# spkelle2/simple_mip_solver

Hardware: AMD Instinct MI355X
Metric: node LP-relaxations/s (higher is better)
Workload: dtype f64

## Files before the change

simple_mip_solver_amd/csrc/lp_kernel.hip.h:

```cpp
#pragma once
#include <type_traits>
#include <hip/hip_runtime.h>
#include <stdint.h>

namespace mipx {

constexpr double kPTol = 1e-7;
constexpr double kDTol = 1e-7;
constexpr double kPivTol = 1e-9;
constexpr double kBTol = 1e-9;
constexpr double kMReport = 1e10;

struct LpArgs {
    int m = 0, n = 0;
    const double *A = nullptr, *b = nullptr, *c = nullptr;
    size_t A_stride = 0, b_stride = 0, c_stride = 0;
    const double *l = nullptr, *u = nullptr;
    const int8_t *vstat_in = nullptr;
    const int32_t *slot = nullptr;
    const double *anchor_T = nullptr, *anchor_vec = nullptr;
    const int32_t *anchor_idx = nullptr;
    const int32_t *anchor_sel = nullptr;
    const double *atab_T = nullptr, *atab_vec = nullptr;
    const int32_t *atab_idx = nullptr;
// ... 192 lines not shown
    const unsigned lm = wave_min_u32(hi == hm ? lo : 0xffffffffu);
    kmin = __hiloint2double((int)hm, (int)lm);
    return wave_pick(valid & (hi == hm) & (lo == lm), payload);
}
__device__ __forceinline__ double uniform_f64(double v) {
    const int lo = __builtin_amdgcn_readfirstlane(__double2loint(v));
    const int hi = __builtin_amdgcn_readfirstlane(__double2hiint(v));
    return __hiloint2double(hi, lo);
}
__device__ __forceinline__ double readlane_f64(double v, int l) {
    const int lo = __builtin_amdgcn_readlane(__double2loint(v), l);
    const int hi = __builtin_amdgcn_readlane(__double2hiint(v), l);
    return __hiloint2double(hi, lo);
}
__device__ __forceinline__ double swz16_f64(double v) {
    const int lo = __builtin_amdgcn_ds_swizzle(__double2loint(v), 0x401f);
    const int hi = __builtin_amdgcn_ds_swizzle(__double2hiint(v), 0x401f);
    return __hiloint2double(hi, lo);
}
__device__ __forceinline__ double xor32_f64(double v) { return __shfl_xor(v, 32, 64); }
__device__ __forceinline__ double xor8_f64(double v) { return dpp_f64<0x128, 0xf>(v); }
__device__ __forceinline__ double xor4_f64(double v) {
    int lo = __builtin_amdgcn_update_dpp(__double2loint(v), __double2loint(v), 0x104, 0xf, 0x5, false);
    int hi = __builtin_amdgcn_update_dpp(__double2hiint(v), __double2hiint(v), 0x104, 0xf, 0x5, false);
    lo = __builtin_amdgcn_update_dpp(lo, __double2loint(v), 0x114, 0xf, 0xa, false);
    hi = __builtin_amdgcn_update_dpp(hi, __double2hiint(v), 0x114, 0xf, 0xa, false);
    return __hiloint2double(hi, lo);
}
__device__ __forceinline__ double xor2_f64(double v) { return dpp_f64<0x4e, 0xf>(v); }
__device__ __forceinline__ double xor1_f64(double v) { return dpp_f64<0xb1, 0xf>(v); }
#define MIPX_ROWSUM_STEP(arr_, h_, dist_, xch_)                                             \
    do {                                                                                    \
        const bool up_ = (lane & (dist_)) != 0;                                             \
        _Pragma("unroll") for (int k_ = 0; k_ < (h_); k_++) {                               \
            const double send_ = up_ ? arr_[k_] : arr_[k_ + (h_)];                          \
            const double keep_ = up_ ? arr_[k_ + (h_)] : arr_[k_];                          \
            arr_[k_] = keep_ + xch_(send_);                                                 \
        }                                                                                   \
    } while (0)
#define MIPX_ROWSUMS(arr_, rp_)                                                             \
    do {                                                                                    \
        if ((rp_) == 32) {                                                                  \
            MIPX_ROWSUM_STEP(arr_, 16, 32, xor32_f64);                                      \
            MIPX_ROWSUM_STEP(arr_, 8, 16, swz16_f64);                                       \
            MIPX_ROWSUM_STEP(arr_, 4, 8, xor8_f64);                                         \
            MIPX_ROWSUM_STEP(arr_, 2, 4, xor4_f64);                                         \
            MIPX_ROWSUM_STEP(arr_, 1, 2, xor2_f64);                                         \
            arr_[0] = arr_[0] + xor1_f64(arr_[0]);                                          \
        } else {                                                                            \
            MIPX_ROWSUM_STEP(arr_, 8, 32, xor32_f64);                                       \
            MIPX_ROWSUM_STEP(arr_, 4, 16, swz16_f64);                                       \
            MIPX_ROWSUM_STEP(arr_, 2, 8, xor8_f64);                                         \
            MIPX_ROWSUM_STEP(arr_, 1, 4, xor4_f64);                                         \
            arr_[0] = arr_[0] + xor2_f64(arr_[0]);                                          \
            arr_[0] = arr_[0] + xor1_f64(arr_[0]);                                          \
        }                                                                                   \
    } while (0)
__device__ __forceinline__ int rowsum_row(int lane, int rp) {
    const int r16 = ((lane & 32) ? 8 : 0) | ((lane & 16) ? 4 : 0) | ((lane & 8) ? 2 : 0) | ((lane & 4) ? 1 : 0);
    return rp == 32 ? 2 * r16 + ((lane & 2) ? 1 : 0) : r16;
}

struct alignas(16) MailA {
    int win;
    int lvmeta;
    double x;
};
struct alignas(16) MailB {
    int q;
    int ev;
    double pinv;
};

template <int NW, int R, int C, int MP>
struct Smem {
    static constexpr int NP = 16 * C;
    alignas(16) double row[NP];
    double alpha[4 * NW * R];
    double lo[NP];
    double up[NP];
    double va[NP];
    double vb[NP];
    double d[NP];
    double key[NP];
    double cvec[NP];
    double beta0[MP];
    double ba[4 * NW * R];
    double bb[4 * NW * R];
    double wgt[4 * NW * R];
    double tau[4 * NW * R];
    MailA mbA;
    MailB mbB;
    int bvar[MP];
    int meta[NP];
    int nvar[NP];
    int side[NP];
    int wlist[NP];
    int nw;
    int nfake0;
    double objv;
    int dive_code;
    int seq;
    int pos[NP + MP];
    int8_t wantb[NP + MP];
    int8_t atup[NP + MP];
#ifdef MIPX_KPROF
    unsigned long long prof[16];
#endif
};
__device__ __forceinline__ void read_mail(const MailA &mb, int &win, int &lvmeta, double &x) {
    const int4 v = *reinterpret_cast<const int4 *>(&mb);
    win = __builtin_amdgcn_readfirstlane(v.x);
    lvmeta = __builtin_amdgcn_readfirstlane(v.y);
    x = __hiloint2double(__builtin_amdgcn_readfirstlane(v.w), __builtin_amdgcn_readfirstlane(v.z));
}
__device__ __forceinline__ void read_mail(const MailB &mb, int &q, int &ev, double &pinv) {
    const int4 v = *reinterpret_cast<const int4 *>(&mb);
    q = __builtin_amdgcn_readfirstlane(v.x);
    ev = __builtin_amdgcn_readfirstlane(v.y);
    pinv = __hiloint2double(__builtin_amdgcn_readfirstlane(v.w), __builtin_amdgcn_readfirstlane(v.z));
}

#define MIPX_PICK(dst_, arr_, n_, k_)                                                       \
    do {                                                                                    \
        dst_ = arr_[0];                                                                     \
        _Pragma("unroll") for (int t_ = 1; t_ < n_; t_++) dst_ = (k_) == t_ ? arr_[t_] : dst_; \
    } while (0)
template <int C>
struct RowArr {
    double v[C];
    __device__ __forceinline__ double &operator[](int j) { return v[j]; }
    __device__ __forceinline__ const double &operator[](int j) const { return v[j]; }
};
#define MIPX_ROW(ii_) (grp + NG * (ii_))
#define MIPX_COL(jj_) (32 * ((jj_) >> 1) + 2 * cl + ((jj_)&1))
#define MIPX_PUBLISH_COL(q_)                                                                \
    do {                                                                                    \
        const int qjj_ = 2 * ((q_) >> 5) + ((q_)&1);                                        \
        if (cl == (((q_)&31) >> 1)) {                                                       \
            if constexpr (kVecT) {                                                          \
                _Pragma("unroll") for (int ii = 0; ii < R; ii++) s.alpha[MIPX_ROW(ii)] = T[ii][qjj_]; \
            } else {                                                                        \
                _Pragma("unroll") for (int jj = 0; jj < C; jj++) if (jj == qjj_) {          \
                    _Pragma("unroll") for (int ii = 0; ii < R; ii++) s.alpha[MIPX_ROW(ii)] = T[ii][jj]; \
                }                                                                           \
            }                                                                               \
        }                                                                                   \
         \
         \
        if (lane == 0) __hip_atomic_fetch_add(&s.seq, 1, __ATOMIC_RELEASE, __HIP_MEMORY_SCOPE_WORKGROUP); \
        __builtin_amdgcn_fence(__ATOMIC_RELEASE, "wavefront");                              \
        __builtin_amdgcn_wave_barrier();                                                    \
        __builtin_amdgcn_fence(__ATOMIC_ACQUIRE, "wavefront");                              \
        _Pragma("unroll") for (int ii = 0; ii < R; ii++) al[ii] = s.alpha[MIPX_ROW(ii)];    \
    } while (0)
#define MIPX_AWAIT_COL(target_)                                                             \
    do {                                                                                    \
        while (__hip_atomic_load(&s.seq, __ATOMIC_ACQUIRE, __HIP_MEMORY_SCOPE_WORKGROUP) < (target_)) \
            __builtin_amdgcn_s_sleep(1);                                                    \
    } while (0)
#define MIPX_EXTRACT_ROW(r_)                                                                \
    do {                                                                                    \
        const int rl_ = (r_) / NG;                                                          \
        if (grp == (r_) % NG) {                                                             \
            _Pragma("unroll") for (int ii = 0; ii < R; ii++) if (ii == rl_) {               \
                _Pragma("unroll") for (int jj = 0; jj < C; jj++) s.row[MIPX_COL(jj)] = T[ii][jj]; \
            }                                                                               \
        }                                                                                   \
    } while (0)
#define MIPX_ROW_LDS(jj_) s.row[MIPX_COL(jj_)]
#define MIPX_ROW_REG(jj_) rw[jj_]
#define MIPX_UPDATE_T(r_, q_, pinv_, rowsrc_)                                               \
    do {                                                                                    \
        const int rg_ = (r_) % NG, rl_ = (r_) / NG;                                         \
        const int qcl_ = ((q_)&31) >> 1, qjj_ = 2 * ((q_) >> 5) + ((q_)&1);                 \
        double rh[C];                                                                       \
        _Pragma("unroll") for (int jj = 0; jj < C; jj++) rh[jj] = rowsrc_(jj) * (pinv_);    \
        _Pragma("unroll") for (int ii = 0; ii < R; ii++) {                                  \
            _Pragma("unroll") for (int jj = 0; jj < C; jj++)                                \
                T[ii][jj] = fma(-al[ii], rh[jj], T[ii][jj]);                                \
        }                                                                                   \
        if (cl == qcl_) {                                   \
            if constexpr (kVecT) {                                                          \
                _Pragma("unroll") for (int ii = 0; ii < R; ii++) T[ii][qjj_] = -al[ii] * (pinv_); \
// ... 270 lines not shown
        const double *rowp[R];
#pragma unroll
        for (int ii = 0; ii < R; ii++) {
            const int r = min(MIPX_ROW(ii), m > 0 ? m - 1 : 0);
            if (CUTS && r >= m0) rowp[ii] = g.cut_pi + (size_t)cids[r - m0] * n;
            else rowp[ii] = tsrc + (size_t)r * n;
        }
        if ((n & 1) == 0 && n >= 2) {
            int poff[C / 2];
#pragma unroll
            for (int pp = 0; pp < C / 2; pp++) poff[pp] = min(32 * pp + 2 * cl, n - 2);
#pragma unroll
            for (int ii = 0; ii < R; ii++) {
                const double *arow = rowp[ii];
#pragma unroll
                for (int pp = 0; pp < C / 2; pp++) {
                    const double2 v = m > 0 ? *reinterpret_cast<const double2 *>(arow + poff[pp]) : double2{0.0, 0.0};
                    T[ii][2 * pp] = v.x;
                    T[ii][2 * pp + 1] = v.y;
                }
            }
        } else {
#pragma unroll
            for (int ii = 0; ii < R; ii++) {
                const double *arow = rowp[ii];
#pragma unroll
                for (int jj = 0; jj < C; jj++) T[ii][jj] = m > 0 ? arow[min(MIPX_COL(jj), n - 1)] : 0.0;
            }
        }
    }
    {
        static_assert(NT >= NP + MP, "one staging element per thread");
        const int ic = min(tid, m > 0 ? m - 1 : 0), jc = min(tid, n - 1), vc = min(tid, nv - 1);
        double g_b0;
        if (CUTS && ic >= m0) g_b0 = g.cut_pi0[cids[ic - m0]];
        else g_b0 = anchored ? avec[n + ic] : (m > 0 ? gb[ic] : 0.0);
        const int g_bv = anchored ? aidx[n + ic] : n + ic;
        const double g_d = anchored ? avec[jc] : gc[jc];
        const int g_nv = anchored ? aidx[jc] : jc;
        const double g_lo = lk[jc], g_up = uk[jc];
        const double g_c = gc[jc];
        const int8_t g_st = vin ? vin[vc] : (int8_t)0;
        if (tid < MP) {
            s.beta0[tid] = tid < m ? (anchored ? g_b0 : -g_b0) : 0.0;
            s.bvar[tid] = tid < m ? g_bv : -1;
        }
        if (tid < NP) {
            s.d[tid] = tid < n ? g_d : 0.0;
            s.nvar[tid] = tid < n ? g_nv : -1;
            s.lo[tid] = tid < n ? g_lo : 0.0;
            s.up[tid] = tid < n ? g_up : 0.0;
            s.va[tid] = 0.0;
            s.vb[tid] = 0.0;
            s.cvec[tid] = tid < n ? g_c : 0.0;
        }
        if (tid < NP + MP) {
            const int8_t st = tid < nv ? g_st : (int8_t)0;
            s.wantb[tid] = st == 1;
            s.atup[tid] = st == 2;
            s.pos[tid] = -1;
        }
    }
    int ci[PJ];
    bool cv[PJ], che[PJ];
    double ccl[PJ], ccr[PJ];
#pragma unroll
    for (int kk = 0; kk < PJ; kk++) { ci[kk] = 0; cv[kk] = false; che[kk] = true; ccl[kk] = 0.0; ccr[kk] = 0.0; }
    if (DIVE && ctl && g.dive) {
#pragma unroll
        for (int kk = 0; kk < PJ; kk++) {
            const int k = lane + 64 * kk;
            cv[kk] = k < g.n_int;
            ci[kk] = g.int_idx[cv[kk] ? k : 0];
        }
        if (g.rule != 0) {
#pragma unroll
            for (int kk = 0; kk < PJ; kk++) {
                che[kk] = g.has_entry[ci[kk]] != 0;
                ccl[kk] = g.cost_l[ci[kk]];
                ccr[kk] = g.cost_r[ci[kk]];
            }
        }
    }
    if (tid == 0) s.seq = 0;
    if (DIVE && g.dive_preset && tid < g.dive) {
        g.status[(size_t)node + (size_t)(tid + 1) * (size_t)g.dive_off] = -1;
        g.dive_var[(size_t)tid * (size_t)g.dive_off + node] = -1;
    }
    if (g.zero16 != nullptr && node == 0 && tid < 4) g.zero16[tid] = 0;
    KPROF_SETUP_MARK(9);
    __syncthreads();
    KPROF_SETUP_MARK(10);
    for (int j = tid; j < NP; j += NT) {
        const int v = s.nvar[j];
        if (j < n) s.pos[v] = j;
        const bool fix = j < n && v < n && s.lo[v < n && v >= 0 ? v : 0] == s.up[v < n && v >= 0 ? v : 0];
        s.meta[j] = (v << 3) | (fix ? 4 : 0);
    }
    __syncthreads();
    KPROF_SETUP_MARK(12);
    if (tid < 64) {
        int cnt = 0;
        for (int base = 0; base < nv; base += 64) {
            const int v = base + lane;
            const bool w = v < nv && s.wantb[v] && s.pos[v] >= 0;
            const unsigned long long mask = __ballot(w);
            if (w) s.wlist[cnt + __popcll(mask & ((1ull << lane) - 1ull))] = s.pos[v];
            cnt += __popcll(mask);
        }
        if (lane == 0) s.nw = cnt;
    }
#pragma unroll
    for (int kk = 0; kk < PJ; kk++) {
        cD[kk] = s.d[lane + 64 * kk];
        cM[kk] = s.meta[lane + 64 * kk];
    }
#pragma unroll
    for (int kk = 0; kk < PI; kk++) {
        const int i = lane + 64 * kk;
        const int ic = i < MP ? i : 0;
        const int v = i < MP ? s.bvar[ic] : -1;
        const bool st = v >= 0 && v < n;
        rB0[kk] = i < MP ? s.beta0[ic] : 0.0;
        rBa[kk] = 0.0;
        rBb[kk] = 0.0;
        rW[kk] = 1.0;
        rLo[kk] = st ? s.lo[st ? v : 0] : 0.0;
        rUp[kk] = st ? s.up[st ? v : 0] : INF;
        rM[kk] = (v << 2) | ((v >= 0 && s.wantb[v < 0 ? 0 : v]) ? 1 : 0);
    }
    KPROF_SETUP_MARK(13);
    __syncthreads();
    const int nw = __builtin_amdgcn_readfirstlane(s.nw);
    if (!ctl) {
#pragma unroll
        for (int ii = 0; ii < R; ii++) {
#pragma unroll
            for (int jj = 0; jj < C; jj++)
                T[ii][jj] = (MIPX_ROW(ii) < m && MIPX_COL(jj) < n) ? sgn * T[ii][jj] : 0.0;
        }
    }

    int npiv = 0, iters = 0, status = -1;
    const int cap = 100 * (m + n) + 1000;
    int cols = 0;
    KPROF_MARK(15);

    if (vin) {
        if (ctl) {
            for (int w = 0; w < nw; w++) {
                const int q = __builtin_amdgcn_readfirstlane(s.wlist[w]);
                cols++;
                MIPX_AWAIT_COL(NW * cols);
                double k1 = -1.0, k2 = -1.0;
                int p1 = kNoCand, p2 = kNoCand;
                double rc[PI], av[PI];
#pragma unroll
                for (int kk = 0; kk < PI; kk++) {
                    const int i = lane + 64 * kk;
                    av[kk] = i < MP ? s.alpha[i < MP ? i : 0] : 0.0;
                    const double a = fabs(av[kk]);
                    const bool ok = i < m && a > kPivTol;
                    const bool wanted = rM[kk] & 1, ent = rM[kk] & 2;
                    rc[kk] = 1.0 / av[kk];
                    keep_max(k1, p1, a, i, ok & !wanted);
                    keep_max(k2, p2, a, i, ok & wanted & !ent);
                }
// ... 138 lines not shown
                for (int jj = 0; jj < C; jj++) va[jj] = s.vb[MIPX_COL(jj)];
#pragma unroll
                for (int ii = 0; ii < R; ii++) {
                    double t[C];
#pragma unroll
                    for (int jj = 0; jj < C; jj++) t[jj] = T[ii][jj] * va[jj];
#pragma unroll
                    for (int h = C / 4; h >= 1; h >>= 1) {
#pragma unroll
                        for (int k = 0; k < 2 * h; k++) t[k] = t[k] + t[k + 2 * h];
                    }
                    s0[ii] = t[0];
                    s1[ii] = t[1];
                }
#pragma unroll
                for (int ii = 0; ii < R; ii++) {
                    s0[ii] = s0[ii] + dpp_f64<0x108, 0xf>(s0[ii]);
                    s1[ii] = s1[ii] + dpp_f64<0x108, 0xf>(s1[ii]);
                    s0[ii] = s0[ii] + dpp_f64<0x104, 0xf>(s0[ii]);
                    s1[ii] = s1[ii] + dpp_f64<0x104, 0xf>(s1[ii]);
                    s0[ii] = s0[ii] + dpp_f64<0x102, 0xf>(s0[ii]);
                    s1[ii] = s1[ii] + dpp_f64<0x102, 0xf>(s1[ii]);
                    s0[ii] = s0[ii] + dpp_f64<0x101, 0xf>(s0[ii]);
                    s1[ii] = s1[ii] + dpp_f64<0x101, 0xf>(s1[ii]);
                }
                if (cl == 0) {
#pragma unroll
                    for (int ii = 0; ii < R; ii++) s.bb[MIPX_ROW(ii)] = snap_m(0.0 - (s0[ii] + s1[ii]));
                }
            }
            MIPX_EXACT_WEIGHTS();
        }
        __syncthreads();
        KPROF_MARK(7);
    }

    int pass = 0;
    asm volatile("" : "+s"(pass));
    size_t onode = (size_t)node;
    bool symU = false;
    int dvar = -1, ddir = 0;
    double dbound = 0.0;
    int wage = 0;
#pragma clang loop unroll(disable)
    for (;;) {
    if (solve) {
        if (ctl) {
            bool bland = false;
            int degen = 0;
            const int nfk0 = nfake;
            int nfk = nfk0;
            if (pass == 0) symU = nfake != 0;
            double dje[PJ], cN[PJ];
            unsigned cS[PJ];
            int cP[PJ];
            int cF[PJ];
            double sel_b0 = 0.0, sel_ba = 0.0, sel_bb = 0.0;
            double sel_w = 1.0;
            int sel_win = 0, sel_lvmeta = 0;
            double sel_la = 0.0;
            if (pass == 0) {
#pragma unroll
                for (int kk = 0; kk < PI; kk++) {
                    const int i = lane + 64 * kk;
                    rBa[kk] = i < MP ? rB0[kk] - s.ba[i < MP ? i : 0] : 0.0;
                    rBb[kk] = i < MP ? s.bb[i < MP ? i : 0] : 0.0;
                    rW[kk] = i < MP ? s.wgt[i < MP ? i : 0] : 1.0;
                }
            } else {
#pragma unroll
                for (int kk = 0; kk < PI; kk++) {
                    const bool hit = (rM[kk] >> 2) == dvar;
                    rUp[kk] = (hit && ddir == 0) ? dbound : rUp[kk];
                    rLo[kk] = (hit && ddir != 0) ? dbound : rLo[kk];
                }
                if (lane == 0) {
                    if (ddir == 0) s.up[dvar] = dbound;
                    else s.lo[dvar] = dbound;
                }
            }
            constexpr bool kShadow = NW >= 7;
            MIPX_LEAVE_SELECT();
            if constexpr (!kShadow) MIPX_LEAVE_FETCH();
            __syncthreads();
            for (;;) {
                if (sel_win >> 16) { const int cmd = sel_win >> 16; status = cmd == 1 ? 0 : cmd == 3 ? 2 : 3; break; }
                const int r = sel_win & 0x7fff;
                const unsigned sflip = (sel_win & 0x8000) ? 0x80000000u : 0u;
                if constexpr (kShadow) {
                    MIPX_LEAVE_FETCH();
                    MIPX_PREP_COLS();
                }
                KPROF_MARK(1);
                __syncthreads();
                KPROF_RT_MARK(8);
                if constexpr (!kShadow) MIPX_PREP_COLS();
                double aa[PJ];
                bool el[PJ];
                double k1 = INF;
                int p1 = kNoCand;
#pragma unroll
                for (int kk = 0; kk < PJ; kk++) {
                    const double rv = s.row[lane + 64 * kk];
                    const double a = __hiloint2double(__double2hiint(rv) ^ (sflip ^ cS[kk]), __double2loint(rv));
                    el[kk] = (cF[kk] == 0) & (a > kPivTol);
                    aa[kk] = fabs(a);
                }
                double key[PJ];
#pragma unroll
                for (int kk = 0; kk < PJ; kk++) key[kk] = cN[kk] / aa[kk];
#pragma unroll
                for (int kk = 0; kk < PJ; kk++) keep_min(k1, p1, key[kk], cP[kk], el[kk]);
                KPROF_RT_PIN_D(k1); KPROF_RT_PIN_D(p1);
                KPROF_RT_MARK(9);
                double thmax;
                const int w1 = wave_argmin_pos(k1, p1, thmax);
                KPROF_RT_PIN_I(w1); KPROF_RT_PIN_D(thmax);
                KPROF_RT_MARK(10);
                int qq = -1;
                if (w1 != kNoCand && bland) {
                    qq = w1 & 0xffff;
                } else if (w1 != kNoCand) {
                    const int jmin = w1 & 0xffff;
                    double k2 = -1.0;
                    int p2 = kNoCand;
#pragma unroll
                    for (int kk = 0; kk < PJ; kk++) {
                        const int j = lane + 64 * kk;
                        const bool ok = el[kk] & ((j == jmin) | !(dje[kk] > thmax * aa[kk]));
                        keep_max(k2, p2, aa[kk], cP[kk], ok);
                    }
                    KPROF_RT_PIN_D(k2); KPROF_RT_PIN_D(p2);
                    KPROF_RT_MARK(12);
                    double amax;
                    qq = wave_argmax_pos(k2, p2, amax) & 0xffff;
                    KPROF_RT_PIN_I(qq);
                    KPROF_RT_MARK(13);
                }
                if (lane == 0) s.mbB.q = qq;
                KPROF_RT_PIN_I(qq);
                KPROF_RT_MARK(14);
                KPROF_MARK(3);
                __syncthreads();
                if (qq < 0) { status = 1; break; }
                const int q = qq;
                const int lvmeta = sel_lvmeta;
                const double la = sel_la, lb = (lvmeta & 3) == 2 ? 1.0 : 0.0;
                int ev;
                double vaq, vbq;
                {
                    const int ql = qq & 63, qk = qq >> 6;
                    double t0;
                    int tm;
                    MIPX_PICK(t0, dje, PJ, qk);
                    MIPX_PICK(tm, cM, PJ, qk);
                    const double djq = readlane_f64(t0, ql);
                    const int cm = __builtin_amdgcn_readlane(tm, ql);
                    degen = djq <= kDTol ? degen + 1 : 0;
                    bland = degen > m + n;
                    nfk += ((lvmeta & 3) == 2 ? 1 : 0) - ((cm & 3) == 2 ? 1 : 0);
                    symU |= ((lvmeta & 3) == 2) | ((cm & 3) == 2);
                    ev = cm >> 3;
                    vaq = uniform_f64(s.va[qq]);
                    vbq = uniform_f64(s.vb[qq]);
                }
                const double pinv = 1.0 / uniform_f64(s.row[q]);
// ... 37 lines not shown
                        rUp[kk] = pr ? eup : rUp[kk];
                    }
                    if (++wage == kDseRefresh) {
                        wage = 0;
                        __syncthreads();
#pragma unroll
                        for (int kk = 0; kk < PI; kk++) rW[kk] = lane + 64 * kk < MP ? s.wgt[lane + 64 * kk < MP ? lane + 64 * kk : 0] : 1.0;
                    }
                    MIPX_LEAVE_SELECT();
                    if constexpr (!kShadow) MIPX_LEAVE_FETCH();
                }
                KPROF_MARK(5);
                __syncthreads();
                KPROF_MARK(0);
            }
            (void)nfk0;
            nfake = nfk;
        } else {
            __syncthreads();
            for (;;) {
                int win, lvmeta;
                double la;
                read_mail(s.mbA, win, lvmeta, la);
                if (win >> 16) break;
                const int r = win & 0x7fff;
                MIPX_EXTRACT_ROW(r);
                KPROF_MARK(1);
                __syncthreads();
                double rw[C];
#pragma unroll
                for (int jj = 0; jj < C; jj++) rw[jj] = s.row[MIPX_COL(jj)];
                {
                    double tq[R];
                    MIPX_ROW_FOLD(MIPX_TERM_ROW, tq);
                    if (cl == 0) {
#pragma unroll
                        for (int ii = 0; ii < R; ii++) s.tau[MIPX_ROW(ii)] = tq[ii];
                    }
                }
                __syncthreads();
                KPROF_MARK(3);
                int q, ev;
                double pinv;
                read_mail(s.mbB, q, ev, pinv);
                if (q < 0) break;
                KPROF_MARK(8);
                MIPX_PUBLISH_COL(q);
                pinv = 1.0 / uniform_f64(s.row[q]);
                KPROF_MARK(4);
                MIPX_UPDATE_T(r, q, pinv, MIPX_ROW_REG);
                if (++wage == kDseRefresh) {
                    wage = 0;
                    MIPX_EXACT_WEIGHTS();
                    __syncthreads();
                }
                KPROF_MARK(5);
                __syncthreads();
                KPROF_MARK(0);
            }
        }
    } else {
        status = 3;
    }

    int o_tid = tid, o_lane = lane, o_n = n, o_m = m;
    asm volatile("" : "+v"(o_tid), "+v"(o_lane), "+s"(o_n), "+s"(o_m));
    {
    const int tid = o_tid, lane = o_lane, n = o_n, m = o_m;
    const int ms = CUTS ? g.mstride : o_m;
#ifdef MIPX_KPROF
    KPROF_MARK(6);
    __syncthreads();
    if (g.prof && tid == 0) {
        for (int k = 0; k < 16; k++) { atomicAdd(&g.prof[k], s.prof[k]); s.prof[k] = 0; }
        atomicAdd(&g.prof[16], (unsigned long long)iters);
        atomicAdd(&g.prof[17], (unsigned long long)(npiv - iters));
        atomicAdd(&g.prof[18], 1ull);
    }
    __syncthreads();
    tprev = clock64();
#endif
    if (g.y == nullptr && g.dbg_T == nullptr) {
    const bool more = DIVE && pass < g.dive && solve;
    if (ctl) {
        constexpr int PER = NP / 64;
        static_assert(PER == PJ, "one column per lane and slot");
#pragma unroll
        for (int kk = 0; kk < PJ; kk++) {
            const int j = lane + 64 * kk;
            const int v = cM[kk] >> 3, sd = cM[kk] & 3;
            if (j >= n) s.key[j] = 0.0;
            if (j < n && v < n) s.key[v] = sd == 2 ? kMReport : s.va[j];
        }
#pragma unroll
        for (int kk = 0; kk < PI; kk++) {
            const int i = lane + 64 * kk;
            const int v = rM[kk] >> 2;
            if (i < m && v < n) s.key[v] = fma(rBb[kk], kMReport, rBa[kk]);
        }
        if (g.vstat_out) {
            int8_t *vo = g.vstat_out + onode * (size_t)(n + ms);
#pragma unroll
            for (int kk = 0; kk < PI; kk++)
                if (lane + 64 * kk < m) vo[rM[kk] >> 2] = 1;
#pragma unroll
            for (int kk = 0; kk < PJ; kk++)
                if (lane + 64 * kk < n) vo[cM[kk] >> 3] = (cM[kk] & 3) ? 2 : 3;
        }
        double p[PER];
#pragma unroll
        for (int k = 0; k < PER; k++) {
            const int j = lane + 64 * k;
            const double xj = s.key[j];
            if (g.x && j < n) g.x[onode * n + j] = xj;
            p[k] = j < n ? s.cvec[j] * xj : 0.0;
        }
#pragma unroll
        for (int h = PER / 2; h >= 1; h >>= 1) {
#pragma unroll
            for (int k = 0; k < h; k++) p[k] = p[k] + p[k + h];
        }
        double sum = p[0];
        sum = sum + xor32_f64(sum);
        sum = sum + swz16_f64(sum);
        sum = sum + xor8_f64(sum);
        sum = sum + xor4_f64(sum);
        sum = sum + xor2_f64(sum);
        sum = sum + xor1_f64(sum);
        const double objv = uniform_f64(sum);
        int code = -1;
        double dval = 0.0;
        if (more && status == 0 && objv < g.dive_cutoff) {
            double bk = -1.0;
            int bp = kNoCand, nprobe = 0;
#pragma unroll
            for (int kk = 0; kk < PJ; kk++) {
                const int k = lane + 64 * kk;
                const double v = s.key[ci[kk]];
                const double fl = floor(v), ce = ceil(v);
                const double dist = fmin(v - fl, ce - v);
                const bool frac = cv[kk] && dist > kVarEps;
                const double key = g.rule == 0 ? dist : fmin(ccr[kk] * (ce - v), ccl[kk] * (v - fl));
                keep_max(bk, bp, key, k, frac && che[kk]);
                nprobe += __popcll(__ballot(frac && !che[kk]));
            }
            double km;
            const int win = wave_argmax_pos(bk, bp, km);
            if (win != kNoCand && nprobe == 0) {
                const int wl = win & 63, wk = win >> 6;
                int t_i;
                double t_l, t_r;
                MIPX_PICK(t_i, ci, PJ, wk);
                MIPX_PICK(t_l, ccl, PJ, wk);
                MIPX_PICK(t_r, ccr, PJ, wk);
                dvar = __builtin_amdgcn_readlane(t_i, wl);
                const double wcl = readlane_f64(t_l, wl), wcr = readlane_f64(t_r, wl);
                const double v = uniform_f64(s.key[dvar]);
                const double fl = floor(v), ce = ceil(v);
                if (g.rule == 0) ddir = (v - fl <= ce - v) ? 0 : 1;
                else ddir = (wcl * (v - fl) <= wcr * (ce - v)) ? 0 : 1;
                dbound = ddir == 0 ? fl : ce;
                dval = v;
                bool mine = false;
#pragma unroll
                for (int kk = 0; kk < PI; kk++) mine |= (lane + 64 * kk < m) && (rM[kk] >> 2) == dvar;
                if (__ballot(mine) != 0ull) code = dvar;
            }
        }
        if (lane == 0) {
            if (g.obj) g.obj[onode] = status == 1 ? INF : objv;
            if (g.status) g.status[onode] = status;
            if (g.iters) g.iters[onode] = iters;
            if (g.npivots) g.npivots[onode] = npiv;
            if (code >= 0) {
                const size_t di = (size_t)pass * (size_t)g.dive_off + node;
                g.dive_var[di] = dvar;
                g.dive_dir[di] = ddir;
                g.dive_val[di] = dval;
            }
            s.dive_code = code;
        }
    }
    if (!more) break;
    KPROF_OUT_MARK(14);
    __syncthreads();
    } else {
    if (ctl) {
#pragma unroll
        for (int kk = 0; kk < PJ; kk++) {
            const int j = lane + 64 * kk;
            const int v = cM[kk] >> 3, sd = cM[kk] & 3;
            s.d[j] = cD[kk];
            s.nvar[j] = v;
            s.side[j] = sd;
            if (j < n && v < n) s.key[v] = sd == 2 ? kMReport : s.va[j];
        }
#pragma unroll
        for (int kk = 0; kk < PI; kk++) {
            const int i = lane + 64 * kk;
            if (i < MP) {
                const int v = rM[kk] >> 2;
                s.beta0[i] = rB0[kk];
                s.ba[i] = rBa[kk];
                s.bb[i] = rBb[kk];
                s.bvar[i] = v;
                if (i < m && v < n) s.key[v] = fma(rBb[kk], kMReport, rBa[kk]);
            }
        }
    }
    for (int j = n + tid; j < NP; j += NT) s.key[j] = 0.0;
    __syncthreads();
    KPROF_OUT_MARK(9);
    if (g.x)
        for (int j = tid; j < n; j += NT) g.x[onode * n + j] = s.key[j];
    if (g.y) {
        for (int i = tid; i < m; i += NT) g.y[onode * ms + i] = 0.0;
        __syncthreads();
        for (int j = tid; j < n; j += NT)
            if (s.nvar[j] >= n) g.y[onode * ms + (s.nvar[j] - n)] = s.d[j];
    }
    if (g.vstat_out) {
        int8_t *vo = g.vstat_out + onode * (size_t)(n + ms);
        for (int i = tid; i < m; i += NT) vo[s.bvar[i]] = 1;
        for (int j = tid; j < n; j += NT) vo[s.nvar[j]] = s.side[j] ? 2 : 3;
    }
    if (g.dbg_T && (node == 0 || g.dbg_all)) {
        const size_t k = g.dbg_all ? (size_t)node : 0;
        double *dT = g.dbg_T + k * (size_t)ms * n;
        double *dvec = g.dbg_vec + k * (size_t)(n + 3 * ms);
        int32_t *didx = g.dbg_idx + k * (size_t)(2 * n + ms);
#pragma unroll
        for (int ii = 0; ii < R; ii++) {
#pragma unroll
            for (int jj = 0; jj < C; jj++) {
                const int i = MIPX_ROW(ii), j = MIPX_COL(jj);
                if (!ctl && i < m && j < n) dT[(size_t)i * n + j] = T[ii][jj];
            }
        }
        for (int j = tid; j < n; j += NT) {
            dvec[j] = s.d[j];
            didx[j] = s.nvar[j];
            didx[n + m + j] = s.side[j];
        }
        for (int i = tid; i < m; i += NT) {
            dvec[n + i] = s.beta0[i];
            dvec[n + m + i] = s.ba[i];
            dvec[n + 2 * m + i] = s.bb[i];
            didx[n + i] = s.bvar[i];
        }
    }
    KPROF_OUT_MARK(10);
    if (!ctl && tw == 0) {
        constexpr int PER = NP / 64;
        double p[PER];
#pragma unroll
        for (int k = 0; k < PER; k++) {
            const int j = lane + 64 * k;
            p[k] = j < n ? s.cvec[j] * s.key[j] : 0.0;
        }
#pragma unroll
        for (int h = PER / 2; h >= 1; h >>= 1) {
#pragma unroll
            for (int k = 0; k < h; k++) p[k] = p[k] + p[k + h];
        }
        double sum = p[0];
        sum = sum + xor32_f64(sum);
        sum = sum + swz16_f64(sum);
        sum = sum + xor8_f64(sum);
        sum = sum + xor4_f64(sum);
        sum = sum + xor2_f64(sum);
        sum = sum + xor1_f64(sum);
        if (lane == 0) s.objv = sum;
    }
    const bool more = DIVE && pass < g.dive && solve;
    int code = -1;
    double dval = 0.0;
    if (ctl && more && status == 0) {
        double bk = -1.0;
        int bp = kNoCand, nprobe = 0;
#pragma unroll
        for (int kk = 0; kk < PJ; kk++) {
            const int k = lane + 64 * kk;
            const double v = s.key[ci[kk]];
            const double fl = floor(v), ce = ceil(v);
            const double dist = fmin(v - fl, ce - v);
            const bool frac = cv[kk] && dist > kVarEps;
            const double key = g.rule == 0 ? dist : fmin(ccr[kk] * (ce - v), ccl[kk] * (v - fl));
            keep_max(bk, bp, key, k, frac && che[kk]);
            nprobe += __popcll(__ballot(frac && !che[kk]));
        }
        double km;
        const int win = wave_argmax_pos(bk, bp, km);
        if (win != kNoCand && nprobe == 0) {
            const int wl = win & 63, wk = win >> 6;
            int t_i;
            double t_l, t_r;
            MIPX_PICK(t_i, ci, PJ, wk);
            MIPX_PICK(t_l, ccl, PJ, wk);
            MIPX_PICK(t_r, ccr, PJ, wk);
            dvar = __builtin_amdgcn_readlane(t_i, wl);
            const double wcl = readlane_f64(t_l, wl), wcr = readlane_f64(t_r, wl);
            const double v = uniform_f64(s.key[dvar]);
            const double fl = floor(v), ce = ceil(v);
            if (g.rule == 0) ddir = (v - fl <= ce - v) ? 0 : 1;
            else ddir = (wcl * (v - fl) <= wcr * (ce - v)) ? 0 : 1;
            dbound = ddir == 0 ? fl : ce;
            dval = v;
            bool mine = false;
#pragma unroll
            for (int kk = 0; kk < PI; kk++) mine |= (lane + 64 * kk < m) && (rM[kk] >> 2) == dvar;
            if (__ballot(mine) != 0ull) code = dvar;
        }
    }
    KPROF_OUT_MARK(12);
    __syncthreads();
    KPROF_OUT_MARK(13);
    if (ctl) {
        const double objv = uniform_f64(s.objv);
        if (!(status == 0 && objv < g.dive_cutoff)) code = -1;
        if (lane == 0) {
            if (g.obj) g.obj[onode] = status == 1 ? INF : objv;
            if (g.status) g.status[onode] = status;
            if (g.iters) g.iters[onode] = iters;
            if (g.npivots) g.npivots[onode] = npiv;
            if (code >= 0) {
                const size_t di = (size_t)pass * (size_t)g.dive_off + node;
                g.dive_var[di] = dvar;
                g.dive_dir[di] = ddir;
                g.dive_val[di] = dval;
            }
            s.dive_code = code;
        }
    }
    if (!more) break;
    KPROF_OUT_MARK(14);
    __syncthreads();
    }
    }
    if (__builtin_amdgcn_readfirstlane(s.dive_code) < 0) break;
    KPROF_MARK(11);
    pass++;
    onode += (size_t)g.dive_off;
    iters = 0;
    npiv = 0;
    }
}

template <int NW, int R, int C, int MP, bool DIVE = false, bool CUTS = false>
__global__ __launch_bounds__(64 * (NW + 1)) void lp_dual_simplex(LpArgs g) {
    __shared__ Smem<NW, R, C, MP> s;
    if (threadIdx.x < 64) lp_dual_simplex_role<NW, R, C, MP, DIVE, true, CUTS>(g, s);
    else lp_dual_simplex_role<NW, R, C, MP, DIVE, false, CUTS>(g, s);
}

#undef MIPX_PUBLISH_COL
#undef MIPX_PUBLISH_NEXT_COL
#undef MIPX_READ_COL
#undef MIPX_AWAIT_COL
#undef MIPX_EXTRACT_ROW
#undef MIPX_UPDATE_T
#undef MIPX_UPDATE_COLS
#undef MIPX_PREP_COLS
#undef MIPX_PICK
#undef MIPX_ROWSUMS
#undef MIPX_ROWSUM_STEP
#undef MIPX_ROW
#undef MIPX_COL
#undef MIPX_LEAVE_SELECT
#undef MIPX_LEAVE_FETCH
#undef MIPX_ROW_FOLD
#undef MIPX_TERM_SQ
#undef MIPX_TERM_ROW
#undef MIPX_EXACT_WEIGHTS
#undef MIPX_ROW_LDS
#undef MIPX_ROW_REG

}
```

simple_mip_solver_amd/csrc/mipx.hip:

```cpp
#include <hip/hip_runtime.h>

#include <cstdio>
#include <cstdlib>
#include <cstring>
#include <new>
#include <string>
#include <vector>

#include "../../include/mipx.h"
#include "lp_kernel.hip.h"
#include "lp_kernel_big.hip.h"
#include "lp_kernel_root.hip.h"

struct mipx_ctx {
    int device = -1;
    hipStream_t stream = nullptr;
    hipEvent_t ev0 = nullptr, ev1 = nullptr;
    hipEvent_t k0 = nullptr, k1 = nullptr;
    float last_kernel_ms = -1.f;
    std::string err;
    void *scratch = nullptr;
    size_t scratch_bytes = 0;
};

// ... 84 lines not shown
    int RPB = 1;
    while (RPB < 8 && (m + RPB - 1) / RPB > gmax) RPB *= 2;
    const int G = (m + RPB - 1) / RPB;
    if (G > 256) return MIPX_OK;
    const size_t nn = (size_t)n, mm = (size_t)m;
    size_t off = 0;
    auto carve = [&](size_t bytes) { size_t o = off; off = align_up(off + bytes, 256); return o; };
    const size_t o_T = carve(mm * nn * 8), o_b0 = carve(mm * 8), o_ba = carve(mm * 8), o_bb = carve(mm * 8),
                 o_w = carve(mm * 8), o_rl = carve(mm * 8), o_ru = carve(mm * 8), o_bv = carve(mm * 4), o_d = carve(2 * nn * 8), o_va = carve(2 * nn * 8),
                 o_vb = carve(2 * nn * 8), o_nv = carve(2 * nn * 4), o_sd = carve(2 * nn * 4),
                 o_ck = carve(2 * (size_t)G * sizeof(mipx::RootKey)), o_cr = carve(2 * (size_t)G * sizeof(mipx::RootRow)), o_row = carve(2 * (size_t)G * nn * 8),
                 o_ctl = carve(16 * 4);
    if (p->root_state_bytes < off) {
        if (p->root_state) (void)hipFree(p->root_state);
        p->root_state = nullptr; p->root_state_bytes = 0;
        HIP_TRY(ctx, hipMalloc((void **)&p->root_state, off));
        p->root_state_bytes = off;
    }
    char *base = p->root_state;
    mipx::RootState S;
    S.m = m; S.n = n; S.G = G; S.RPB = RPB;
    S.T = (double *)(base + o_T); S.beta0 = (double *)(base + o_b0); S.ba = (double *)(base + o_ba);
    S.bb = (double *)(base + o_bb); S.wgt = (double *)(base + o_w); S.bvar = (int *)(base + o_bv);
    S.rlo = (double *)(base + o_rl); S.rup = (double *)(base + o_ru);
    S.d = (double *)(base + o_d); S.va = (double *)(base + o_va); S.vb = (double *)(base + o_vb);
    S.nvar = (int *)(base + o_nv); S.side = (int *)(base + o_sd);
    S.ckey = (mipx::RootKey *)(base + o_ck); S.crow = (mipx::RootRow *)(base + o_cr); S.rowbuf = (double *)(base + o_row); S.ctl = (int *)(base + o_ctl);
    S.lo = a.l + (size_t)src * nn; S.up = a.u + (size_t)src * nn;
    S.max_iter = a.max_iter; S.cap = 100 * (m + n) + 1000;
    hipLaunchKernelGGL(mipx::lp_root_init, dim3(G), dim3(mipx::kRootNT), 2 * nn * 8, stream, S, a.A, a.b, a.c);
    HIP_TRY(ctx, hipGetLastError());
    int par = 0;
    const int chunk = 192;
    void (*pivot)(mipx::RootState, int) = RPB == 1 ? mipx::lp_root_pivot<1> : RPB == 2 ? mipx::lp_root_pivot<2>
                                           : RPB == 4 ? mipx::lp_root_pivot<4> : mipx::lp_root_pivot<8>;
    const long limit = (long)S.cap + 8;
    for (long done_pivots = 0; done_pivots <= limit; done_pivots += chunk) {
        for (int k = 0; k < chunk; k++, par ^= 1)
            hipLaunchKernelGGL(pivot, dim3(G), dim3(mipx::kRootNT), 0, stream, S, par);
        HIP_TRY(ctx, hipGetLastError());
        int32_t st = -1;
        HIP_TRY(ctx, hipMemcpyAsync(&st, S.ctl + 8 * par, 4, hipMemcpyDeviceToHost, stream));
        HIP_TRY(ctx, hipStreamSynchronize(stream));
        if (st == -2) {
            hipLaunchKernelGGL(mipx::lp_root_values, dim3(G), dim3(mipx::kRootNT), 2 * nn * 8, stream, S, par);
            HIP_TRY(ctx, hipGetLastError());
            par ^= 1;
        }
        if (st >= 0) break;
    }
    hipLaunchKernelGGL(mipx::lp_root_final, dim3(1), dim3(mipx::kRootNT), nn * 8, stream, S, par, a, (size_t)0);
    HIP_TRY(ctx, hipGetLastError());
    *done = true;
    return MIPX_OK;
}

int launch_lp_any(mipx_problem *p, mipx::LpArgs &a, int batch, hipStream_t stream = nullptr, int m_rows = -1) {
    mipx_ctx *ctx = p->ctx;
    if (!stream) stream = ctx->stream;
    if (m_rows < 0) m_rows = p->m;
    if (const KernelCfg *cfg = pick_cfg(m_rows, p->n)) {
#ifdef MIPX_KPROF
        static unsigned long long *d_prof = nullptr;
        if (!d_prof) HIP_TRY(ctx, hipMalloc((void **)&d_prof, 32 * 8));
        HIP_TRY(ctx, hipMemsetAsync(d_prof, 0, 32 * 8, stream));
        a.prof = d_prof;
        a.prof_wave = getenv("MIPX_KPROF_WAVE") ? atoi(getenv("MIPX_KPROF_WAVE")) : 0;
        cfg->launch(a, batch, stream);
        HIP_TRY(ctx, hipStreamSynchronize(stream));
        unsigned long long h[32];
        HIP_TRY(ctx, hipMemcpy(h, d_prof, sizeof h, hipMemcpyDeviceToHost));
        if (getenv("MIPX_KPROF_PRINT")) {
            const double it = h[16] ? (double)h[16] : 1.0, rf = h[17] ? (double)h[17] : 1.0;
            const double lps = h[18] ? (double)h[18] : 1.0;
            fprintf(stderr, "[kprof] %s batch %d wave %d  lps %llu iters %llu refactor pivots %llu\n"
                    "  simplex cycles/iter: m1 %.0f m3 %.0f m2 %.0f m4 %.0f m5 %.0f m0 %.0f  (sum %.0f)\n"
                    "  refactor cycles/pivot: m9 %.0f m10 %.0f m12 %.0f m13 %.0f m14 %.0f  (sum %.0f)\n"
                    "  per LP: setup %.0f m8/iter %.0f m11/iter %.0f value-init %.0f tail %.0f\n",
                    cfg->name, batch, a.prof_wave, h[18], h[16], h[17], h[1] / it, h[3] / it, h[2] / it,
                    h[4] / it, h[5] / it, h[0] / it, (h[0] + h[1] + h[2] + h[3] + h[4] + h[5]) / it,
                    h[9] / rf, h[10] / rf, h[12] / rf, h[13] / rf, h[14] / rf,
                    (h[9] + h[10] + h[12] + h[13] + h[14]) / rf, h[15] / lps, h[8] / it, h[11] / it,
                    h[7] / lps, h[6] / lps);
#ifdef MIPX_KPROF_RT
            fprintf(stderr, "  ratio test cycles/iter: wait at B %.0f pass1 %.0f argmin %.0f pass2 %.0f argmax %.0f tail %.0f  (m3 = the barrier C)\n",
                    h[8] / it, h[9] / it, h[10] / it, h[12] / it, h[13] / it, h[14] / it);
#endif
        }
        return MIPX_OK;
#else
        a.prof = nullptr;
        a.prof_wave = 0;
        cfg->launch(a, batch, stream);
        HIP_TRY(ctx, hipGetLastError());
        return MIPX_OK;
#endif
    }
    {
        bool done = false;
        const int rrc = launch_root_coop(p, a, stream, &done);
        if (rrc || done) return rrc;
    }
    const int mcap = a.ncut ? a.mstride : p->m;
    if (mcap < m_rows || !big_fits(mcap, p->n)) return fail(ctx, MIPX_ETOOBIG, "(m,n) exceeds every LP kernel");
    const bool side = stream != ctx->stream;
    const int cap = side ? 256 : 1024;
    const int slabs = batch < cap ? batch : cap;
    double *&scratch = side ? p->big_scratch2 : p->big_scratch;
    int &have = side ? p->big_slabs2 : p->big_slabs;
    if (mcap > p->big_rows) {
        have = 0;
        if (!side) p->big_slabs2 = 0; else p->big_slabs = 0;
        p->big_rows = mcap;
    }
    if (slabs > have) {
        if (side) HIP_TRY(ctx, hipStreamSynchronize(stream));
        if (scratch) (void)hipFree(scratch);
        scratch = nullptr;
        have = 0;
        HIP_TRY(ctx, hipMalloc((void **)&scratch, (size_t)slabs * p->big_rows * p->n * sizeof(double)));
        have = slabs;
    }
    const size_t lds = mipx::big_lds_bytes(mcap, p->n);
    HIP_TRY(ctx, hipFuncSetAttribute((const void *)mipx::lp_dual_simplex_big,
                                     hipFuncAttributeMaxDynamicSharedMemorySize, (int)lds));
    hipLaunchKernelGGL(mipx::lp_dual_simplex_big, dim3(slabs), dim3(mipx::kBigNT), lds, stream,
                       a, scratch);
    HIP_TRY(ctx, hipGetLastError());
    return MIPX_OK;
}

mipx::LpArgs problem_args(const mipx_problem *p, bool anchor = true) {
    mipx::LpArgs a;
    a.m = p->m; a.n = p->n;
    a.A = p->dA; a.b = p->db; a.c = p->dc;
    if (anchor && p->anchor_on) { a.anchor_T = p->anchor_T; a.anchor_vec = p->anchor_vec; a.anchor_idx = p->anchor_idx; }
    return a;
}

struct Staging {
    struct Copy { void *host; size_t o, bytes; };
    mipx_ctx *ctx;
    const char *who;
    size_t off = 0;
    char *base = nullptr;
    bool own = false;
    std::vector<Copy> ups, downs;

    Staging(mipx_ctx *c, const char *name) : ctx(c), who(name) {}
    int err(const char *what, hipError_t e) { return fail(ctx, MIPX_EHIP, (std::string(who) + ": " + what).c_str(), e); }
    size_t carve(size_t bytes) { const size_t o = off; off = align_up(off + bytes, 256); return o; }
    void up(size_t o, const void *src, size_t bytes) { if (src) ups.push_back({(void *)src, o, bytes}); }
    void down(void *dst, size_t o, size_t bytes) { if (dst) downs.push_back({dst, o, bytes}); }
    size_t in(const void *src, size_t bytes) { const size_t o = carve(bytes); up(o, src, bytes); return o; }
    size_t out(void *dst, size_t bytes) { const size_t o = carve(bytes); down(dst, o, bytes); return o; }
    template <class T> T *at(size_t o) const { return (T *)(base + o); }
    int alloc(void *&block, size_t &have) {
        if (off > have) {
            if (block) (void)hipFree(block);
            block = nullptr;
            have = 0;
            if (hipError_t e = hipMalloc(&block, off)) return err("hipMalloc", e);
            have = off;
        }
        base = (char *)block;
        return MIPX_OK;
// ... 725 lines not shown
```

Measured before the change: 11.45 million.

## Offload LP output epilogue to worker waves and overlap objective with dive selection

The per-LP output phase, once done entirely by the control wave, is now split. The control wave stages x and vstat into shared memory, publishes a sequence flag and picks the dive variable. Worker wave 0 spins on the flag and computes the objective dot product in parallel, and after a barrier the worker waves write x, vstat and the scalar results to global memory using vectorized stores. This is meant to shorten the serial epilogue between dive passes, at the cost of extra shared memory, a spin-wait and the dive candidate now being chosen before the objective cutoff check.

```diff
diff --git a/simple_mip_solver_amd/csrc/lp_kernel.hip.h b/simple_mip_solver_amd/csrc/lp_kernel.hip.h
--- a/simple_mip_solver_amd/csrc/lp_kernel.hip.h
+++ b/simple_mip_solver_amd/csrc/lp_kernel.hip.h
@@ -298,7 +298,7 @@
     double va[NP];
     double vb[NP];
     double d[NP];
-    double key[NP];
+    alignas(16) double key[NP];
     double cvec[NP];
     double beta0[MP];
     double ba[4 * NW * R];
@@ -316,6 +316,10 @@
     int nfake0;
     double objv;
     int dive_code;
+    int xseq;
+    alignas(16) int8_t vst[NP + MP];
+    int ostatus, oiters, onpiv, odvar, oddir;
+    double odval;
     int seq;
     int pos[NP + MP];
     int8_t wantb[NP + MP];
@@ -752,7 +756,7 @@
             }
         }
     }
-    if (tid == 0) s.seq = 0;
+    if (tid == 0) { s.seq = 0; s.xseq = 0; }
     if (DIVE && g.dive_preset && tid < g.dive) {
         g.status[(size_t)node + (size_t)(tid + 1) * (size_t)g.dive_off] = -1;
         g.dive_var[(size_t)tid * (size_t)g.dive_off + node] = -1;
@@ -1057,6 +1061,7 @@
             constexpr bool kShadow = NW >= 7;
             MIPX_LEAVE_SELECT();
             if constexpr (!kShadow) MIPX_LEAVE_FETCH();
+            KPROF_OUT_MARK(13);
             __syncthreads();
             for (;;) {
                 if (sel_win >> 16) { const int cmd = sel_win >> 16; status = cmd == 1 ? 0 : cmd == 3 ? 2 : 3; break; }
@@ -1260,8 +1265,8 @@
 #endif
     if (g.y == nullptr && g.dbg_T == nullptr) {
     const bool more = DIVE && pass < g.dive && solve;
+    constexpr int PER = NP / 64;
     if (ctl) {
-        constexpr int PER = NP / 64;
         static_assert(PER == PJ, "one column per lane and slot");
 #pragma unroll
         for (int kk = 0; kk < PJ; kk++) {
@@ -1276,22 +1281,81 @@
             const int v = rM[kk] >> 2;
             if (i < m && v < n) s.key[v] = fma(rBb[kk], kMReport, rBa[kk]);
         }
+        if (lane == 0) __hip_atomic_store(&s.xseq, pass + 1, __ATOMIC_RELEASE, __HIP_MEMORY_SCOPE_WORKGROUP);
+        double cx[PJ];
+#pragma unroll
+        for (int kk = 0; kk < PJ; kk++) cx[kk] = s.key[ci[kk]];
         if (g.vstat_out) {
-            int8_t *vo = g.vstat_out + onode * (size_t)(n + ms);
 #pragma unroll
             for (int kk = 0; kk < PI; kk++)
-                if (lane + 64 * kk < m) vo[rM[kk] >> 2] = 1;
+                if (lane + 64 * kk < m) s.vst[rM[kk] >> 2] = 1;
 #pragma unroll
             for (int kk = 0; kk < PJ; kk++)
-                if (lane + 64 * kk < n) vo[cM[kk] >> 3] = (cM[kk] & 3) ? 2 : 3;
-        }
+                if (lane + 64 * kk < n) s.vst[cM[kk] >> 3] = (cM[kk] & 3) ? 2 : 3;
+        }
+        if (lane == 0) {
+            s.ostatus = status;
+            s.oiters = iters;
+            s.onpiv = npiv;
+        }
+        KPROF_OUT_MARK(9);
+        int code = -1;
+        double dval = 0.0;
+        if (more && status == 0) {
+            double bk = -1.0;
+            int bp = kNoCand;
+            bool probe = false;
+#pragma unroll
+            for (int kk = 0; kk < PJ; kk++) {
+                const int k = lane + 64 * kk;
+                const double v = cx[kk];
+                const double fl = floor(v), ce = ceil(v);
+                const double dist = fmin(v - fl, ce - v);
+                const bool frac = cv[kk] && dist > kVarEps;
+                const double key = g.rule == 0 ? dist : fmin(ccr[kk] * (ce - v), ccl[kk] * (v - fl));
+                keep_max(bk, bp, key, k, frac && che[kk]);
+                probe |= frac && !che[kk];
+            }
+            double km;
+            const int win = wave_argmax_pos(bk, bp, km);
+            if (win != kNoCand && __ballot(probe) == 0ull) {
+                const int wl = win & 63, wk = win >> 6;
+                int t_i;
+                double t_l, t_r, t_v;
+                MIPX_PICK(t_i, ci, PJ, wk);
+                MIPX_PICK(t_l, ccl, PJ, wk);
+                MIPX_PICK(t_r, ccr, PJ, wk);
+                MIPX_PICK(t_v, cx, PJ, wk);
+                dvar = __builtin_amdgcn_readlane(t_i, wl);
+                const double wcl = readlane_f64(t_l, wl), wcr = readlane_f64(t_r, wl);
+                const double v = readlane_f64(t_v, wl);
+                const double fl = floor(v), ce = ceil(v);
+                if (g.rule == 0) ddir = (v - fl <= ce - v) ? 0 : 1;
+                else ddir = (wcl * (v - fl) <= wcr * (ce - v)) ? 0 : 1;
+                dbound = ddir == 0 ? fl : ce;
+                dval = v;
+                bool mine = false;
+#pragma unroll
+                for (int kk = 0; kk < PI; kk++) mine |= (lane + 64 * kk < m) && (rM[kk] >> 2) == dvar;
+                if (__ballot(mine) != 0ull) code = dvar;
+            }
+        }
+        KPROF_OUT_MARK(12);
+        if (lane == 0) {
+            s.dive_code = code;
+            s.odvar = dvar;
+            s.oddir = ddir;
+            s.odval = dval;
+        }
+    } else if (tw == 0) {
+        while (__hip_atomic_load(&s.xseq, __ATOMIC_ACQUIRE, __HIP_MEMORY_SCOPE_WORKGROUP) <= pass)
+            __builtin_amdgcn_s_sleep(1);
+        KPROF_OUT_MARK(9);
         double p[PER];
 #pragma unroll
         for (int k = 0; k < PER; k++) {
             const int j = lane + 64 * k;
-            const double xj = s.key[j];
-            if (g.x && j < n) g.x[onode * n + j] = xj;
-            p[k] = j < n ? s.cvec[j] * xj : 0.0;
+            p[k] = j < n ? s.cvec[j] * s.key[j] : 0.0;
         }
 #pragma unroll
         for (int h = PER / 2; h >= 1; h >>= 1) {
@@ -1305,63 +1369,73 @@
         sum = sum + xor4_f64(sum);
         sum = sum + xor2_f64(sum);
         sum = sum + xor1_f64(sum);
-        const double objv = uniform_f64(sum);
-        int code = -1;
-        double dval = 0.0;
-        if (more && status == 0 && objv < g.dive_cutoff) {
-            double bk = -1.0;
-            int bp = kNoCand, nprobe = 0;
-#pragma unroll
-            for (int kk = 0; kk < PJ; kk++) {
-                const int k = lane + 64 * kk;
-                const double v = s.key[ci[kk]];
-                const double fl = floor(v), ce = ceil(v);
-                const double dist = fmin(v - fl, ce - v);
-                const bool frac = cv[kk] && dist > kVarEps;
-                const double key = g.rule == 0 ? dist : fmin(ccr[kk] * (ce - v), ccl[kk] * (v - fl));
-                keep_max(bk, bp, key, k, frac && che[kk]);
-                nprobe += __popcll(__ballot(frac && !che[kk]));
-            }
-            double km;
-            const int win = wave_argmax_pos(bk, bp, km);
-            if (win != kNoCand && nprobe == 0) {
-                const int wl = win & 63, wk = win >> 6;
-                int t_i;
-                double t_l, t_r;
-                MIPX_PICK(t_i, ci, PJ, wk);
-                MIPX_PICK(t_l, ccl, PJ, wk);
-                MIPX_PICK(t_r, ccr, PJ, wk);
-                dvar = __builtin_amdgcn_readlane(t_i, wl);
-                const double wcl = readlane_f64(t_l, wl), wcr = readlane_f64(t_r, wl);
-                const double v = uniform_f64(s.key[dvar]);
-                const double fl = floor(v), ce = ceil(v);
-                if (g.rule == 0) ddir = (v - fl <= ce - v) ? 0 : 1;
-                else ddir = (wcl * (v - fl) <= wcr * (ce - v)) ? 0 : 1;
-                dbound = ddir == 0 ? fl : ce;
-                dval = v;
-                bool mine = false;
-#pragma unroll
-                for (int kk = 0; kk < PI; kk++) mine |= (lane + 64 * kk < m) && (rM[kk] >> 2) == dvar;
-                if (__ballot(mine) != 0ull) code = dvar;
-            }
-        }
-        if (lane == 0) {
-            if (g.obj) g.obj[onode] = status == 1 ? INF : objv;
-            if (g.status) g.status[onode] = status;
-            if (g.iters) g.iters[onode] = iters;
-            if (g.npivots) g.npivots[onode] = npiv;
-            if (code >= 0) {
-                const size_t di = (size_t)pass * (size_t)g.dive_off + node;
-                g.dive_var[di] = dvar;
-                g.dive_dir[di] = ddir;
-                g.dive_val[di] = dval;
-            }
-            s.dive_code = code;
-        }
-    }
-    if (!more) break;
+        if (lane == 0) s.objv = sum;
+        KPROF_OUT_MARK(10);
+    }
     KPROF_OUT_MARK(14);
     __syncthreads();
+    const double objv = uniform_f64(s.objv);
+    int code = __builtin_amdgcn_readfirstlane(s.dive_code);
+    if (!(objv < g.dive_cutoff)) code = -1;
+    if (!ctl) {
+        auto kp = __builtin_amdgcn_kernarg_segment_ptr();
+        asm volatile("" : "+s"(kp));
+        const LpArgs __attribute__((address_space(4))) *go = (const LpArgs __attribute__((address_space(4))) *)kp;
+        const int ttid = tid - 64;
+        constexpr int NTT = 64 * NW;
+        double *gx = go->x;
+        if (gx) {
+            double *xo = gx + onode * n;
+            if ((n & 1) == 0 && (reinterpret_cast<uintptr_t>(gx) & 15) == 0) {
+#pragma unroll
+                for (int t = 0; t < (NP / 2 + NTT - 1) / NTT; t++) {
+                    const int j = 2 * (ttid + t * NTT);
+                    if (j < n) *reinterpret_cast<double2 *>(xo + j) = *reinterpret_cast<const double2 *>(&s.key[j]);
+                }
+            } else {
+#pragma unroll
+                for (int t = 0; t < (NP + NTT - 1) / NTT; t++) {
+                    const int j = ttid + t * NTT;
+                    if (j < n) xo[j] = s.key[j];
+                }
+            }
+        }
+        const int rt = NTT - 1 - ttid;
+        int8_t *gv = go->vstat_out;
+        if (gv) {
+            int8_t *vo = gv + onode * (size_t)(n + ms);
+            const int nb = n + m;
+            int k0 = 0;
+            if (((n + ms) & 3) == 0 && (reinterpret_cast<uintptr_t>(gv) & 3) == 0) {
+                k0 = nb & ~3;
+#pragma unroll
+                for (int t = 0; t < ((NP + MP) / 4 + NTT - 1) / NTT; t++) {
+                    const int k = 4 * (rt + t * NTT);
+                    if (k < k0) *reinterpret_cast<int32_t *>(vo + k) = *reinterpret_cast<const int32_t *>(&s.vst[k]);
+                }
+            }
+#pragma unroll
+            for (int t = 0; t < (NP + MP + NTT - 1) / NTT; t++) {
+                const int k = k0 + rt + t * NTT;
+                if (k < nb) vo[k] = s.vst[k];
+            }
+        }
+        if (rt == 0) {
+            const int st = s.ostatus;
+            if (go->obj) go->obj[onode] = st == 1 ? INF : objv;
+            if (go->status) go->status[onode] = st;
+            if (go->iters) go->iters[onode] = s.oiters;
+            if (go->npivots) go->npivots[onode] = s.onpiv;
+            if (code >= 0) {
+                const size_t di = (size_t)pass * (size_t)go->dive_off + node;
+                go->dive_var[di] = s.odvar;
+                go->dive_dir[di] = s.oddir;
+                go->dive_val[di] = s.odval;
+            }
+        }
+        KPROF_OUT_MARK(12);
+    }
+    if (!more || code < 0) break;
     } else {
     if (ctl) {
 #pragma unroll
@@ -1513,9 +1587,9 @@
     if (!more) break;
     KPROF_OUT_MARK(14);
     __syncthreads();
-    }
-    }
     if (__builtin_amdgcn_readfirstlane(s.dive_code) < 0) break;
+    }
+    }
     KPROF_MARK(11);
     pass++;
     onode += (size_t)g.dive_off;
diff --git a/simple_mip_solver_amd/csrc/mipx.hip b/simple_mip_solver_amd/csrc/mipx.hip
--- a/simple_mip_solver_amd/csrc/mipx.hip
+++ b/simple_mip_solver_amd/csrc/mipx.hip
@@ -190,6 +190,10 @@
                     h[9] / rf, h[10] / rf, h[12] / rf, h[13] / rf, h[14] / rf,
                     (h[9] + h[10] + h[12] + h[13] + h[14]) / rf, h[15] / lps, h[8] / it, h[11] / it,
                     h[7] / lps, h[6] / lps);
+#ifdef MIPX_KPROF_OUT
+            fprintf(stderr, "  output cycles/LP: m9 %.0f m10 %.0f m12 %.0f m14 %.0f  barrier m11 %.0f  leaving-row select at a pass start m13 %.0f\n",
+                    h[9] / lps, h[10] / lps, h[12] / lps, h[14] / lps, h[11] / lps, h[13] / lps);
+#endif
 #ifdef MIPX_KPROF_RT
             fprintf(stderr, "  ratio test cycles/iter: wait at B %.0f pass1 %.0f argmin %.0f pass2 %.0f argmax %.0f tail %.0f  (m3 = the barrier C)\n",
                     h[8] / it, h[9] / it, h[10] / it, h[12] / it, h[13] / it, h[14] / it);
```

After: 11.76 million, median of 6. Within noise of the previous version (+2.7%).
